# tingliu/glia

Hardware: AMD Instinct MI355X
Metric: region_merges_per_sec (higher is better)
Workload: dtype u32 labels / f32 image / f64 statistics and features

## Files before the change

### glia_amd/csrc/greedy.hip

```cpp
#include <atomic>
#include <cstring>
#include <vector>
#include <limits>
#include <rocprim/device/device_scan.hpp>
#include <rocprim/device/device_radix_sort.hpp>
#include <rocprim/device/device_segmented_radix_sort.hpp>

#include "greedy_common.hpp"

namespace glia {

__global__ void pq_build_level_kernel(PqTree t, int l) {
  const int lane = threadIdx.x & 63;
  uint32_t j = (blockIdx.x * blockDim.x + threadIdx.x) >> 6;
  if (j < t.lv[l].size) (void)pq_recompute_node(t, l, j, lane, true);
}

int pq_setup(DeviceBuffers& buf, PqTree& t, hipStream_t stream) {
  t.nlevels = 0;
  uint32_t n = t.nleaves;
  while (true) {
    n = (n + kFan - 1) / kFan;
    if (t.nlevels >= kMaxLevels) { set_error("greedy: edge table too large"); return GLIA_HMT_ERR_ARG; }
    PqLevel& L = t.lv[t.nlevels++];
// ... 881 lines not shown
          if (tid == 0) { w.cthr = (int)st.wB; w.tsal = __builtin_inf(); w.tseq = ~0ull; }
          full_barrier();
        }
      }
    }
    const int cthr2 = (wn_now + total > st.wcap) ? w.cthr : cthr;
    const double tsal2 = (wn_now + total > st.wcap) ? w.tsal : tsal;
    const unsigned long long tseq2 = (wn_now + total > st.wcap) ? w.tseq : tseq;
    const uint32_t nwork = small ? s.nitems : total;
    WPH(2);

    bool bad = false;
    uint32_t pend_e = kNone, pend_old = kNone;
    for (uint32_t base = 0; base < nwork; base += kGreedyThreads) {
      const uint32_t i = base + tid;
      if (i >= nwork) break;
      FatEntry f0, f1;
      bool h0, h1;
      uint32_t rs;
      if (small) {
        const uint32_t h = s.items[i];
        rs = s.mk[h] - 1u;
        const uint32_t m0 = s.mv0[h], m1 = s.mv1[h];
        s.mk[h] = 0u; s.mv0[h] = 0u; s.mv1[h] = 0u;
        h0 = m0 != 0; h1 = m1 != 0;
        f0 = s.stage[h0 ? m0 - 1u : m1 - 1u]; f1 = s.stage[h1 ? m1 - 1u : m0 - 1u];
      } else {
        const bool side1 = i >= len0;
        const FatEntry fe = st.fpool[side1 ? off1 + (i - len0) : off0 + i];
        if (fe.eid == e || fe.eid == kNone) continue;
        rs = fe.rs;
        if (!side1) {
          const uint32_t m = st.mark1[rs];
          h0 = true; h1 = m != 0; f0 = fe;
          f1 = h1 ? st.fpool[off1 + (m - 1u - len0)] : fe;
        } else {
          if (st.mark0[rs] != 0u) continue;
          h0 = false; h1 = true; f0 = fe; f1 = fe;
        }
      }
      const uint32_t idx = atomicAdd(&s.newcount, 1u);
      const uint32_t newE = (uint32_t)ne + idx;
      atomicOr(&w.touched[par][(rs >> 5) & 63u], 1u << (rs & 31u));
      double first = 0.0;
      int second = 0;
      if (h0) { first += f0.mean * (int)f0.n; second += (int)f0.n; }
      if (h1) { first += f1.mean * (int)f1.n; second += (int)f1.n; }
      first = sdivide(first, (double)second, 0.0);
      if (first == -1.0) bad = true;
      const uint32_t offRs = f0.off, posRs = f0.pos, lenRs = f0.len;
      if (h0 && h1) st.fpool[offRs + f1.pos].eid = kNone;
      const uint32_t cat = rs < r0 ? 0u : (h0 ? 1u : 2u);
      const unsigned long long seq = ((k + 1ull) << 32) | ((unsigned long long)cat << 30) | rs;
      const double sal = -first;
      EdgeRec* pe = &st.er[newE];
      uint4* pq4 = reinterpret_cast<uint4*>(pe);
      pq4[0] = make_uint4(rs, r2, posRs, idx);
      const unsigned long long mb = (unsigned long long)__double_as_longlong(first);
      pq4[1] = make_uint4((uint32_t)mb, (uint32_t)(mb >> 32), (uint32_t)second, kNone);
      pq4[2] = make_uint4(offRs, lenRs, r2off, 0u);
      const unsigned long long sbits = (unsigned long long)__double_as_longlong(sal);
      pq4[3] = make_uint4((uint32_t)sbits, (uint32_t)(sbits >> 32), (uint32_t)seq, (uint32_t)(seq >> 32));
      FatEntry* pa = &st.fpool[offRs + posRs];
      FatEntry a; a.eid = newE; a.rs = r2; a.n = (uint32_t)second; a.pos = idx; a.off = r2off; a.len = 0; a.mean = first;
      *pa = a;
      FatEntry b; b.eid = newE; b.rs = rs; b.n = (uint32_t)second; b.pos = posRs; b.off = offRs; b.len = lenRs; b.mean = first;
      st.fpool[r2off + idx] = b;
      if (small) { s.items[i] = offRs + posRs; s.newidx[i] = idx; }
      const uint32_t cell = win_cell(sal, smin, scale, st.wB);
      if (win_above(cthr2, tsal2, tseq2, (int)cell, sal, seq)) {
        const uint32_t sl = atomicAdd(&w.n, 1u);
        win_put(w, sl, sal, seq, newE, rs, r2, make_uint2(offRs, lenRs), make_uint2(r2off, 0u));
      } else {
        if (pend_e != kNone) st.er[pend_e].next = pend_old;
        pend_e = newE; pend_old = atomicExch(&st.whead[cell], newE);
        atomicAdd(&st.wcnt[cell], 1u);
      }
#pragma unroll
      for (int side = 0; side < 2; ++side) {
        const bool hs = side ? h1 : h0;
        if (!hs) continue;
        const uint32_t de = side ? f1.eid : f0.eid;
        const double dsal = -(side ? f1.mean : f0.mean);
        const uint32_t dc = win_cell(dsal, smin, scale, st.wB);
        unsigned long long dq = 1;
        const bool tie = (int)dc == cthr2 && dsal == tsal2;
        if (COND || tie) dq = st.er[de].seq;
        st.er[de].seq = 0;
        if (dq != 0) {
          if (win_above(cthr2, tsal2, tseq2, (int)dc, dsal, dq)) {
            const uint32_t j = atomicAdd(&w.nk, 1u); if (j < kKillMax) w.kill[j] = de; else w.kovf = 1;
          } else atomicSub(&st.wcnt[dc], 1u);
        }
      }
    }
    if (bad) s.bad = 1;
    if (small) lds_barrier(); else full_barrier();
    if (s.bad) { if (pend_e != kNone) st.er[pend_e].next = pend_old; status = ST_BAD_SALIENCY; break; }
    WPH(3);
    const uint32_t newcount = s.newcount;
    if (small) {
      for (uint32_t i = tid; i < nwork; i += kGreedyThreads) { st.fpool[s.items[i]].len = newcount; st.er[(uint32_t)ne + s.newidx[i]].hv.y = newcount; }
    } else {
      for (uint32_t j = tid; j < newcount; j += kGreedyThreads) {
        const FatEntry fb = st.fpool[r2off + j];
        st.fpool[fb.off + fb.pos].len = newcount;
        st.er[(uint32_t)ne + j].hv.y = newcount;
        st.mark0[fb.rs] = 0; st.mark1[fb.rs] = 0;
      }
    }
    if (w.kovf) full_barrier(); else lds_barrier();
    if (tid == 0) { st.adj_off[r2] = r2off; st.adj_len[r2] = newcount; s.nitems = 0; s.newcount = 0; }
    win_scan(st, w, tid, r2, newcount);
    if (pend_e != kNone) st.er[pend_e].next = pend_old;
    r2prev = r2;
    WPH(4);
#ifdef GLIA_HMT_PROFILE
    if (tid == 0) {
      const unsigned long long tn = __builtin_readcyclecounter();
      const int b = total <= 64 ? 0 : total <= 512 ? 1 : total <= kMarkMax ? 2 : total <= 8192 ? 3 : 4;
      wtb[b] += tn - wtiter; wnb[b] += 1; wdb[b] += total; wtiter = tn; winwin += w.n;
    }
#endif
    k += 1; ne += newcount; pool_used += total;
  }
#ifdef GLIA_HMT_PROFILE
  if (tid == 0) printf("[window profile] merges %llu: pop %llu  lists+table %llu  room %llu  build %llu  finish+scan %llu  loop-top %llu  reload %llu (cycles); reloads %llu (items %llu) compactions %llu dependent %llu; mean window fill %llu\n",
                       k, wph[0], wph[1], wph[2], wph[3], wph[4], wph[5], wph[6], wreloads, wloaded, wcompacts, wdeps, k ? winwin / k : 0ull);
  if (tid == 0) printf("[window profile] by width (<=64, <=512, <=1408, <=8192, more): merges %llu %llu %llu %llu %llu  cycles %llu %llu %llu %llu %llu  entries %llu %llu %llu %llu %llu\n",
                       wnb[0], wnb[1], wnb[2], wnb[3], wnb[4], wtb[0], wtb[1], wtb[2], wtb[3], wtb[4], wdb[0], wdb[1], wdb[2], wdb[3], wdb[4]);
#endif
  full_barrier();
  win_flush(st, w, tid);
  if (tid == 0) {
    st.ctrl[0] = k; st.ctrl[1] = ne; st.ctrl[2] = pool_used; st.ctrl[3] = w.err ? (unsigned long long)ST_INTERNAL : status; st.ctrl[9] = w.err; st.ctrl[10] = w.n;
    st.ctrl[5] = (unsigned long long)(long long)w.cthr; st.ctrl[6] = (unsigned long long)__double_as_longlong(w.tsal); st.ctrl[7] = w.tseq; st.ctrl[8] = w.iptr;
  }
}

constexpr uint32_t kBatchKill = 32;
constexpr int kMemP = 3;
constexpr uint32_t kMemMax = 192;
struct BatchShared {
  alignas(16) Key part1[kNW];
  alignas(16) Key part2[kNW];
  uint32_t nkill, kovf; alignas(16) uint32_t kill[kBatchKill];
  uint32_t byrank[kNW];
  uint32_t bitmap[kNW][64];
  uint32_t m_newcount[kNW], m_total[kNW], m_ok[kNW];
  double m_maxsal[kNW];
  uint32_t bad;
};

#ifdef GLIA_HMT_PROFILE
__device__ unsigned long long g_scanprof[8];
#define SCAN_T(i) do { if (tid == 0) { const unsigned long long tn_ = __builtin_readcyclecounter(); g_scanprof[i] += tn_ - st_; st_ = tn_; } } while (0)
#else
#define SCAN_T(i) do {} while (0)
#endif
__device__ __forceinline__ void batch_scan(const WinState& st, WinShared& w, BatchShared& b, int tid) {
#ifdef GLIA_HMT_PROFILE
  unsigned long long st_ = __builtin_readcyclecounter();
  if (tid == 0) g_scanprof[7] += 1;
#endif
  const uint32_t n = w.n < st.wcap ? w.n : st.wcap, nk = b.nkill < kBatchKill ? b.nkill : kBatchKill, kovf = b.kovf;
  const uint32_t own = 64u * (uint32_t)(((tid >> 6) + (tid & 63)) & 7) + (uint32_t)(tid & 63);
  unsigned long long q[kWinPer]; uint32_t e[kWinPer]; double sl[kWinPer];
#pragma unroll
  for (int j = 0; j < kWinPer; ++j) { const uint32_t i = own + (uint32_t)j * kGreedyThreads; q[j] = w.seq[i]; e[j] = w.e[i]; sl[j] = w.sal[i]; }
  const uint4 ka = *reinterpret_cast<const uint4*>(&b.kill[0]), kb = *reinterpret_cast<const uint4*>(&b.kill[4]);
  const uint32_t kl[8] = {ka.x, ka.y, ka.z, ka.w, kb.x, kb.y, kb.z, kb.w};
  Key k1, k2;
  k1.sal = -__builtin_inf(); k1.seq = 0; k1.arg = 0; k2 = k1;
  SCAN_T(0);
  uint32_t deadm[kWinPer];
#pragma unroll
  for (int j = 0; j < kWinPer; ++j) {
    uint32_t d = 0;
#pragma unroll
    for (uint32_t t = 0; t < 8; ++t) d |= (uint32_t)(t < nk) & (uint32_t)(kl[t] == e[j]);
    deadm[j] = d;
  }
  if (nk > 8u) {
    for (uint32_t t = 8; t < nk; ++t) {
      const uint32_t kt = b.kill[t];
#pragma unroll
      for (int j = 0; j < kWinPer; ++j) deadm[j] |= (uint32_t)(kt == e[j]);
    }
    if (kovf) {
      full_barrier();
#pragma unroll
      for (int j = 0; j < kWinPer; ++j) {
        const uint32_t i = own + (uint32_t)j * kGreedyThreads;
        if (i < n && q[j] != 0) deadm[j] |= (uint32_t)(st.er[e[j]].seq == 0);
      }
    }
  }
#pragma unroll
  for (int j = 0; j < kWinPer; ++j) {
    const uint32_t i = own + (uint32_t)j * kGreedyThreads;
    const bool was = (i < n) & (q[j] != 0);
    const bool live = was & (deadm[j] == 0u);
    if (was & !live) w.seq[i] = 0;
    Key c; c.sal = live ? sl[j] : -__builtin_inf(); c.seq = live ? q[j] : 0ull; c.arg = i;
    const bool b1 = better(c, k1), b2 = better(c, k2);
    k2.sal = b1 ? k1.sal : (b2 ? c.sal : k2.sal); k2.seq = b1 ? k1.seq : (b2 ? c.seq : k2.seq); k2.arg = b1 ? k1.arg : (b2 ? c.arg : k2.arg);
    k1.sal = b1 ? c.sal : k1.sal; k1.seq = b1 ? c.seq : k1.seq; k1.arg = b1 ? c.arg : k1.arg;
  }
  SCAN_T(1);
  const Key m1 = wave_max_sal_first(k1);
  SCAN_T(2);
  const bool mine = (k1.seq == m1.seq) & (k1.arg == m1.arg) & (m1.seq != 0);
  Key kk; kk.sal = mine ? k2.sal : k1.sal; kk.seq = mine ? k2.seq : k1.seq; kk.arg = mine ? k2.arg : k1.arg;
  const Key m2 = wave_max_sal_first(kk);
  SCAN_T(3);
  if ((tid & 63) == 0) { b.part1[tid >> 6] = m1; b.part2[tid >> 6] = m2; }
  full_barrier();
  SCAN_T(4);
  if (tid == 0) { b.nkill = 0; b.kovf = 0; }
}

#ifdef GLIA_HMT_PROFILE
__device__ unsigned long long g_wideprof[8];
#define WIDE_T(i) do { if (tid == 0) { const unsigned long long tn_ = __builtin_readcyclecounter(); g_wideprof[i] += tn_ - wt_; wt_ = tn_; } } while (0)
#else
#define WIDE_T(i) do {} while (0)
#endif
__device__ __forceinline__ uint32_t batch_contract_wide(const WinState& st, WinShared& w, WinWork& s, BatchShared& b, int tid, uint32_t slot, double rootsal,
                                                      unsigned long long k, unsigned long long ne, unsigned long long pool_used, uint32_t* newcount_out) {
  const double smin = st.wrange[0], scale = st.wrange[1];
  const uint32_t e = w.e[slot], r0 = w.u[slot], r1 = w.v[slot];
  const uint2 h0r = w.hu[slot], h1r = w.hv[slot];
  const uint32_t wn_now = w.n;
  const uint32_t off0 = h0r.x, len0 = h0r.y, off1 = h1r.x, len1 = h1r.y;
  const uint32_t total = len0 + len1;
  const uint32_t r2 = st.R0 + (uint32_t)k;
  const uint32_t r2off = (uint32_t)pool_used;
#ifdef GLIA_HMT_PROFILE
  unsigned long long wt_ = __builtin_readcyclecounter();
#endif
  lds_barrier();
  WIDE_T(0);
  if (tid == 0) {
    w.seq[slot] = 0;
    st.order[3 * k + 0] = r0; st.order[3 * k + 1] = r1; st.order[3 * k + 2] = r2;
    st.sal_out[k] = rootsal;
    st.er[e].seq = 0;
    st.rdead[r0] = 1; st.rdead[r1] = 1;
  }
  const bool small = total <= kMarkMax;
  for (uint32_t i = tid; i < total; i += kGreedyThreads) {
    const bool side1 = i >= len0;
    const FatEntry fe = st.fpool[side1 ? off1 + (i - len0) : off0 + i];
    if (fe.eid == e || fe.eid == kNone) continue;
    if (small) {
      s.stage[i] = fe;
      uint32_t h = (fe.rs * 2654435761u) >> 21;
      while (true) {
        const uint32_t old = atomicCAS(&s.mk[h], 0u, fe.rs + 1u);
        if (old == 0u) { s.items[atomicAdd(&s.nitems, 1u)] = h; break; }
        if (old == fe.rs + 1u) break;
        h = (h + 1u) & (kMarkSlots - 1u);
      }
      (side1 ? s.mv1 : s.mv0)[h] = i + 1u;
    } else (side1 ? st.mark1 : st.mark0)[fe.rs] = i + 1u;
  }
  if (small) lds_barrier(); else full_barrier();
  WIDE_T(1);
  if (wn_now + total > st.wcap && wn_now > st.wcap / 2u) win_compact(w, tid, st.wcap);
  WIDE_T(2);
  const int cthr = w.cthr; const double tsal = w.tsal; const unsigned long long tseq = w.tseq;
  const uint32_t nwork = small ? s.nitems : total;
  const uint32_t lenR2 = small ? nwork : 0u;
  bool bad = false;
  uint32_t pend_e = kNone, pend_old = kNone;
  auto rounds = [&](auto small_tag) {
    constexpr bool SMALL = decltype(small_tag)::value;
    for (uint32_t base = 0; base < nwork; base += kGreedyThreads) {
      const uint32_t i = base + tid;
      if (i >= nwork) break;
      FatEntry f0, f1;
      bool h0, h1;
      uint32_t rs;
      if constexpr (SMALL) {
        const uint32_t h = s.items[i];
        rs = s.mk[h] - 1u;
        const uint32_t m0 = s.mv0[h], m1 = s.mv1[h];
        s.mk[h] = 0u; s.mv0[h] = 0u; s.mv1[h] = 0u;
        h0 = m0 != 0; h1 = m1 != 0;
        f0 = s.stage[h0 ? m0 - 1u : m1 - 1u]; f1 = s.stage[h1 ? m1 - 1u : m0 - 1u];
      } else {
        const bool side1 = i >= len0;
        const FatEntry fe = st.fpool[side1 ? off1 + (i - len0) : off0 + i];
        if (fe.eid == e || fe.eid == kNone) continue;
        rs = fe.rs;
        if (!side1) {
          const uint32_t m = st.mark1[rs];
          h0 = true; h1 = m != 0; f0 = fe;
          f1 = h1 ? st.fpool[off1 + (m - 1u - len0)] : fe;
        } else {
          if (st.mark0[rs] != 0u) continue;
          h0 = false; h1 = true; f0 = fe; f1 = fe;
        }
      }
      const uint32_t idx = atomicAdd(&s.newcount, 1u);
      const uint32_t newE = (uint32_t)ne + idx;
      double first = 0.0;
      int second = 0;
      if (h0) { first += f0.mean * (int)f0.n; second += (int)f0.n; }
      if (h1) { first += f1.mean * (int)f1.n; second += (int)f1.n; }
      first = sdivide(first, (double)second, 0.0);
      if (first == -1.0) bad = true;
      const uint32_t offRs = f0.off, posRs = f0.pos, lenRs = f0.len;
      if (h0 && h1) st.fpool[offRs + f1.pos].eid = kNone;
      const uint32_t cat = rs < r0 ? 0u : (h0 ? 1u : 2u);
      const unsigned long long seq = ((k + 1ull) << 32) | ((unsigned long long)cat << 30) | rs;
      const double sal = -first;
      uint4* pq4 = reinterpret_cast<uint4*>(&st.er[newE]);
      pq4[0] = make_uint4(rs, r2, posRs, idx);
      const unsigned long long mb = (unsigned long long)__double_as_longlong(first);
      pq4[1] = make_uint4((uint32_t)mb, (uint32_t)(mb >> 32), (uint32_t)second, kNone);
      pq4[2] = make_uint4(offRs, lenRs, r2off, lenR2);
      const unsigned long long sbits = (unsigned long long)__double_as_longlong(sal);
      pq4[3] = make_uint4((uint32_t)sbits, (uint32_t)(sbits >> 32), (uint32_t)seq, (uint32_t)(seq >> 32));
      FatEntry a; a.eid = newE; a.rs = r2; a.n = (uint32_t)second; a.pos = idx; a.off = r2off; a.len = lenR2; a.mean = first;
      st.fpool[offRs + posRs] = a;
      FatEntry bb; bb.eid = newE; bb.rs = rs; bb.n = (uint32_t)second; bb.pos = posRs; bb.off = offRs; bb.len = lenRs; bb.mean = first;
      st.fpool[r2off + idx] = bb;
      const uint32_t cell = win_cell(sal, smin, scale, st.wB);
      uint32_t sl = kWinCap;
      const bool above = win_above(cthr, tsal, tseq, (int)cell, sal, seq);
      if (above) {
        sl = atomicAdd(&w.n, 1u);
        if (sl < st.wcap) win_put(w, sl, sal, seq, newE, rs, r2, make_uint2(offRs, lenRs), make_uint2(r2off, lenR2));
        else atomicMax(&w.spill_ord, f64_ord(sal));
      }
      if (sl >= st.wcap && (above || cell >= st.wch)) {
        if (pend_e != kNone) st.er[pend_e].next = pend_old;
        pend_e = newE; pend_old = atomicExch(&st.whead[cell], newE);
        atomicAdd(&st.wcnt[cell], 1u);
      }
  #pragma unroll
      for (int side = 0; side < 2; ++side) {
        const bool hs = side ? h1 : h0;
        if (!hs) continue;
        const uint32_t de = side ? f1.eid : f0.eid;
        const double dsal = -(side ? f1.mean : f0.mean);
        const uint32_t dc = win_cell(dsal, smin, scale, st.wB);
        const bool tie = (int)dc == cthr && dsal == tsal;
        if (dc >= st.wch) {
          st.er[de].seq = 0;
          if (tie || win_above(cthr, tsal, tseq, (int)dc, dsal, 0ull)) {
            const uint32_t j = atomicAdd(&b.nkill, 1u); if (j < kBatchKill) b.kill[j] = de; else b.kovf = 1;
          } else atomicSub(&st.wcnt[dc], 1u);
        }
      }
    }
  };
  if (small) rounds(std::true_type{}); else rounds(std::false_type{});
  if (bad) b.bad = 1;
  WIDE_T(3);
  if (small) lds_barrier(); else full_barrier();
  WIDE_T(4);
  const uint32_t newcount = s.newcount;
  if (!small) {
    for (uint32_t j = tid; j < newcount; j += kGreedyThreads) {
      const FatEntry fb = st.fpool[r2off + j];
      st.fpool[fb.off + fb.pos].len = newcount;
      st.er[(uint32_t)ne + j].hv.y = newcount;
      st.mark0[fb.rs] = 0; st.mark1[fb.rs] = 0;
    }
  }
  if (!small) for (uint32_t i = tid; i < (w.n < st.wcap ? w.n : st.wcap); i += kGreedyThreads) if (w.v[i] == r2) w.hv[i].y = newcount;
  if (pend_e != kNone) st.er[pend_e].next = pend_old;
  if (tid == 0) { st.adj_off[r2] = r2off; st.adj_len[r2] = newcount; }
  lds_barrier();
  WIDE_T(5);
  if (tid == 0) { s.nitems = 0; s.newcount = 0; }
  *newcount_out = newcount;
  return total;
}

__global__ __launch_bounds__(kGreedyThreads) void greedy_batch_kernel(WinState st) {
  __shared__ WinShared w;
  __shared__ WinWork s;
  __shared__ BatchShared b;
  const int tid = threadIdx.x, lane = tid & 63, wave = tid >> 6;
  unsigned long long k = st.ctrl[0], ne = st.ctrl[1], pool_used = st.ctrl[2];
  uint32_t status = ST_RUN;
  if (tid == 0) {
    w.n = 0; w.nk = 0; w.kovf = 0; w.err = 0; w.spill_ord = 0; s.nitems = 0; s.newcount = 0; s.bad = 0; b.nkill = 0; b.kovf = 0; b.bad = 0;
    w.cthr = (int)(long long)st.ctrl[5]; w.tsal = __longlong_as_double((long long)st.ctrl[6]); w.tseq = st.ctrl[7]; w.iptr = (uint32_t)st.ctrl[8];
  }
  for (uint32_t i = tid; i < kMarkSlots; i += kGreedyThreads) { s.mk[i] = 0; s.mv0[i] = 0; s.mv1[i] = 0; }
  for (uint32_t i = tid; i < kWinCap; i += kGreedyThreads) { w.seq[i] = 0; w.e[i] = 0; w.v[i] = 0; w.sal[i] = 0.0; }
  b.bitmap[wave][lane] = 0;
  if (tid < kNW) { Key z; z.sal = -__builtin_inf(); z.seq = 0; z.arg = 0; b.part1[tid] = z; b.part2[tid] = z; }
  full_barrier();
  const double smin = st.wrange[0], scale = st.wrange[1];
  uint32_t pend_e = kNone, pend_old = kNone;
  constexpr uint32_t kTab = kMarkSlots / kNW;
  uint32_t* const tk = &s.mk[wave * kTab]; uint32_t* const t0 = &s.mv0[wave * kTab]; uint32_t* const t1 = &s.mv1[wave * kTab];
  static_assert(sizeof(s.stage) >= (size_t)kNW * kTab * 20, "per-wave staging");
  uint32_t* const sg_eid = reinterpret_cast<uint32_t*>(&s.stage[0]) + wave * kTab;
  uint32_t* const sg_n = reinterpret_cast<uint32_t*>(&s.stage[0]) + (kNW + wave) * kTab;
  uint32_t* const sg_pos = reinterpret_cast<uint32_t*>(&s.stage[0]) + (2 * kNW + wave) * kTab;
  double* const sg_mean = reinterpret_cast<double*>(reinterpret_cast<uint32_t*>(&s.stage[0]) + 3 * kNW * kTab) + wave * kTab;
#ifdef GLIA_HMT_PROFILE
  unsigned long long bph[8] = {0, 0, 0, 0, 0, 0, 0, 0}, blast = __builtin_readcyclecounter(), brounds = 0, bmembers = 0, bvalid = 0, bwide = 0, bcut_sal = 0, bcut_dep = 0;
  unsigned long long bw_n[4] = {0, 0, 0, 0}, bw_cyc[4] = {0, 0, 0, 0}, bw_ent[4] = {0, 0, 0, 0}, bw_new[4] = {0, 0, 0, 0};
#define BPH(i) do { if (tid == 0) { unsigned long long tn = __builtin_readcyclecounter(); bph[i] += tn - blast; blast = tn; } } while (0)
#else
#define BPH(i) do {} while (0)
#endif

  for (unsigned long long it = 0; it < st.max_iters; ++it) {
    if (ne - st.ne_base > st.rebase_after) { status = ST_REBASE; break; }
    const int gi = lane >> 3, gj = lane & 7;
    const Key A = b.part1[gi], B = b.part1[gj], C = b.part2[gi];
    const unsigned long long beats = __ballot(better(A, B)), under = __ballot(better(C, B));
    const unsigned long long col = 0x0101010101010101ull << gj;
    const uint32_t rank = (uint32_t)__popcll(beats & col);
    const bool cand_ok = B.seq != 0 && (under & col) == 0;
    if (gi == 0 && cand_ok) b.byrank[rank] = (uint32_t)gj;
    const unsigned long long okmask = __ballot(gi == 0 && cand_ok);
    const uint32_t M = (uint32_t)__popcll(okmask);
    if (M == 0) {
      BPH(5);
      if (pend_e != kNone) { st.er[pend_e].next = pend_old; pend_e = kNone; }
      if (st.force_tree && k >= st.force_tree) { status = ST_NEED_TREE; break; }
      const int r = win_reload(st, w, tid, reinterpret_cast<double*>(&s.stage[0]), reinterpret_cast<unsigned long long*>(&s.stage[0]) + kSelMax);
      BPH(6);
      if (r == 1) { status = ST_DONE; break; }
      if (r == 2) { status = ST_NEED_TREE; break; }
      if (r == 3) { status = ST_REBASE; break; }
      batch_scan(st, w, b, tid);
      continue;
    }
    const unsigned long long minemask = __ballot(gi == 0 && cand_ok && rank == (uint32_t)wave);
    const bool member = minemask != 0;
    const int cj = member ? (int)__builtin_ctzll(minemask) : 0;
    const Key me = b.part1[cj];
    const uint32_t slot = me.arg;
    const uint32_t e = w.e[slot], r0 = w.u[slot], r1 = w.v[slot];
    const uint2 h0r = w.hu[slot], h1r = w.hv[slot];
    const uint32_t off0 = h0r.x, len0 = h0r.y, off1 = h1r.x, len1 = h1r.y;
    const uint32_t total = len0 + len1;
    if (k >= (unsigned long long)st.R0) { status = ST_INTERNAL; break; }
    const unsigned long long firstmask = __ballot(gi == 0 && cand_ok && rank == 0u);
    const Key top = b.part1[__builtin_ctzll(firstmask)];
    const uint2 th0 = w.hu[top.arg], th1 = w.hv[top.arg];
    const uint32_t top_total = th0.y + th1.y;
    BPH(0);
    if (top_total > kMemMax) {
      if (ne + top_total > st.Ecap) { status = ST_NEED_EDGES; break; }
      if (pool_used + top_total > st.pool_cap) { status = ST_NEED_POOL; break; }
      uint32_t newcount = 0;
#ifdef GLIA_HMT_PROFILE
      const unsigned long long tw0 = __builtin_readcyclecounter();
#endif
      const uint32_t tt = batch_contract_wide(st, w, s, b, tid, top.arg, top.sal, k, ne, pool_used, &newcount);
      if (b.bad) { status = ST_BAD_SALIENCY; break; }
      k += 1; ne += newcount; pool_used += tt;
#ifdef GLIA_HMT_PROFILE
      bwide += 1;
      { const int cls = tt <= 512u ? 0 : tt <= kMarkMax ? 1 : tt <= 8192u ? 2 : 3; bw_n[cls] += 1; bw_cyc[cls] += __builtin_readcyclecounter() - tw0; bw_ent[cls] += tt; bw_new[cls] += newcount; }
#endif
      batch_scan(st, w, b, tid);
      if (w.spill_ord) { if (pend_e != kNone) { st.er[pend_e].next = pend_old; pend_e = kNone; } win_evict(st, w, tid); batch_scan(st, w, b, tid); }
      BPH(4);
      continue;
    }
    const bool narrow = member && total <= kMemMax;
    b.bitmap[wave][lane] = 0;
    FatEntry fe[kMemP];
    bool act[kMemP], side1[kMemP];
    uint32_t h[kMemP];
#pragma unroll
    for (int p = 0; p < kMemP; ++p) {
      const uint32_t i = (uint32_t)lane + 64u * (uint32_t)p;
      const bool inlist = narrow && i < total;
      side1[p] = i >= len0;
      fe[p].eid = kNone; fe[p].rs = 0; fe[p].n = 0; fe[p].pos = 0; fe[p].off = 0; fe[p].len = 0; fe[p].mean = 0.0;
      if (inlist) fe[p] = st.fpool[side1[p] ? off1 + (i - len0) : off0 + i];
      act[p] = inlist;
    }
    if (pend_e != kNone) { st.er[pend_e].next = pend_old; pend_e = kNone; }
#pragma unroll
    for (int p = 0; p < kMemP; ++p) {
      act[p] = act[p] && fe[p].eid != e && fe[p].eid != kNone;
      h[p] = (fe[p].rs * 2654435761u) >> 24;
      if (act[p]) {
        while (true) {
          const uint32_t old = atomicCAS(&tk[h[p]], 0u, fe[p].rs + 1u);
          if (old == 0u || old == fe[p].rs + 1u) break;
          h[p] = (h[p] + 1u) & (kTab - 1u);
        }
        if (side1[p]) {
          t1[h[p]] = 1u;
          sg_eid[h[p]] = fe[p].eid; sg_n[h[p]] = fe[p].n; sg_pos[h[p]] = fe[p].pos; sg_mean[h[p]] = fe[p].mean;
        } else t0[h[p]] = 1u;
        atomicOr(&b.bitmap[wave][(fe[p].rs >> 5) & 63u], 1u << (fe[p].rs & 31u));
      }
    }
    if (narrow && lane == 0) { atomicOr(&b.bitmap[wave][(r0 >> 5) & 63u], 1u << (r0 & 31u)); atomicOr(&b.bitmap[wave][(r1 >> 5) & 63u], 1u << (r1 & 31u)); }
    asm volatile("s_waitcnt lgkmcnt(0)" ::: "memory");
    bool owner[kMemP], both[kMemP];
    uint32_t p_eid[kMemP], p_n[kMemP], p_pos[kMemP];
    double p_mean[kMemP];
#pragma unroll
    for (int p = 0; p < kMemP; ++p) {
      const uint32_t m0 = act[p] ? t0[h[p]] : 0u, m1 = act[p] ? t1[h[p]] : 0u;
      owner[p] = act[p] && (!side1[p] || m0 == 0u);
      both[p] = owner[p] && !side1[p] && m1 != 0u;
      p_eid[p] = sg_eid[h[p]]; p_n[p] = sg_n[h[p]]; p_pos[p] = sg_pos[h[p]]; p_mean[p] = sg_mean[h[p]];
    }
#pragma unroll
    for (int p = 0; p < kMemP; ++p) if (act[p]) { tk[h[p]] = 0u; t0[h[p]] = 0u; t1[h[p]] = 0u; }
    double first[kMemP]; int second[kMemP]; uint32_t idx[kMemP];
    bool bad = false;
    uint32_t newcount = 0;
    double mx = -__builtin_inf();
#pragma unroll
    for (int p = 0; p < kMemP; ++p) {
      const bool h0 = owner[p] && !side1[p], h1 = owner[p] && (side1[p] || both[p]);
      double f = 0.0;
      int sc = 0;
      if (h0) { f += fe[p].mean * (int)fe[p].n; sc += (int)fe[p].n; }
      if (h1) { const double m = both[p] ? p_mean[p] : fe[p].mean; const int nn = both[p] ? (int)p_n[p] : (int)fe[p].n; f += m * nn; sc += nn; }
      f = owner[p] ? sdivide(f, (double)sc, 0.0) : 0.0;
      bad = bad || (owner[p] && f == -1.0);
      first[p] = f; second[p] = sc;
      const unsigned long long ownmask = __ballot(owner[p]);
      idx[p] = newcount + (uint32_t)__popcll(ownmask & ((1ull << lane) - 1ull));
      newcount += (uint32_t)__popcll(ownmask);
      mx = (owner[p] && -f > mx) ? -f : mx;
    }
#pragma unroll
    for (int d = 32; d >= 1; d >>= 1) { const double o = __shfl_xor(mx, d); mx = o > mx ? o : mx; }
    if (lane == 0) { b.m_newcount[wave] = narrow ? newcount : 0u; b.m_total[wave] = narrow ? total : 0xFFFFFFFFu; b.m_maxsal[wave] = mx; }
    if (bad) b.bad = 1;
    const uint32_t wn_round = w.n;
    lds_barrier();
    BPH(1);
    if (b.bad) { status = ST_BAD_SALIENCY; break; }
    uint32_t V, ne_off, pool_off, my_ne, my_pool;
    {
      const uint32_t j = (uint32_t)lane & 7u;
      const Key kj = b.part1[b.byrank[j]];
      const uint32_t u = w.u[kj.arg], v = w.v[kj.arg];
      const uint32_t tj = b.m_total[j], nj = b.m_newcount[j];
      double pm = -__builtin_inf();
      uint32_t hit = 0, pre_n = 0, pre_t = 0;
#pragma unroll
      for (uint32_t i = 0; i < (uint32_t)kNW; ++i) {
        const double ms = b.m_maxsal[i];
        const uint32_t bu = b.bitmap[i][(u >> 5) & 63u], bv = b.bitmap[i][(v >> 5) & 63u];
        const uint32_t ti = b.m_total[i], ni = b.m_newcount[i];
        if (i < j) { pm = ms > pm ? ms : pm; hit |= ((bu >> (u & 31u)) | (bv >> (v & 31u))) & 1u; pre_n += ni; pre_t += ti; }
      }
      const bool okj = j < M && tj != 0xFFFFFFFFu && (j == 0u || (kj.sal > pm && hit == 0u));
      const uint32_t okbits = (uint32_t)(__ballot(lane < kNW && okj) & 0xFFull);
      V = (uint32_t)__builtin_ctz(~okbits);
#ifdef GLIA_HMT_PROFILE
      if (V < M) { const uint32_t cutsal = (uint32_t)(__ballot(lane < kNW && j == V && !(kj.sal > pm)) & 0xFFull); if (cutsal) bcut_sal += 1; else bcut_dep += 1; }
#endif
      my_ne = (uint32_t)__builtin_amdgcn_readlane((int)pre_n, wave); my_pool = (uint32_t)__builtin_amdgcn_readlane((int)pre_t, wave);
      const uint32_t last = V - 1u;
      ne_off = (uint32_t)__shfl((int)(pre_n + nj), (int)last); pool_off = (uint32_t)__shfl((int)(pre_t + tj), (int)last);
    }
    const uint32_t sum_tot = pool_off;
    if (ne + sum_tot > st.Ecap) { status = ST_NEED_EDGES; break; }
    if (pool_used + sum_tot > st.pool_cap) { status = ST_NEED_POOL; break; }
    bool popped = false;
    if (wn_round + ne_off > st.wcap && wn_round > st.wcap / 2u) {
      if ((uint32_t)wave < V && lane == 0) w.seq[slot] = 0;
      popped = true;
      lds_barrier();
      win_compact(w, tid, st.wcap);
    }
    const int cthr = w.cthr; const double tsal = w.tsal; const unsigned long long tseq = w.tseq;
    BPH(2);
    if ((uint32_t)wave < V) {
      const unsigned long long kk = k + (unsigned long long)wave;
      const uint32_t r2 = st.R0 + (uint32_t)kk;
      const uint32_t r2off = (uint32_t)pool_used + my_pool;
      if (lane == 0) {
        if (!popped) w.seq[slot] = 0;
        st.order[3 * kk + 0] = r0; st.order[3 * kk + 1] = r1; st.order[3 * kk + 2] = r2;
        st.sal_out[kk] = me.sal;
        st.er[e].seq = 0;
        st.rdead[r0] = 1; st.rdead[r1] = 1;
        st.adj_off[r2] = r2off; st.adj_len[r2] = newcount;
      }
#pragma unroll
      for (int p = 0; p < kMemP; ++p) {
        if (!owner[p]) continue;
        const bool h0 = !side1[p];
        const uint32_t rs = fe[p].rs;
        const uint32_t newE = (uint32_t)ne + my_ne + idx[p];
        const uint32_t offRs = fe[p].off, posRs = fe[p].pos, lenRs = fe[p].len;
        if (both[p]) st.fpool[offRs + p_pos[p]].eid = kNone;
        const uint32_t cat = rs < r0 ? 0u : (h0 ? 1u : 2u);
        const unsigned long long seq = ((kk + 1ull) << 32) | ((unsigned long long)cat << 30) | rs;
        const double sal = -first[p];
        uint4* pq4 = reinterpret_cast<uint4*>(&st.er[newE]);
        pq4[0] = make_uint4(rs, r2, posRs, idx[p]);
        const unsigned long long mb = (unsigned long long)__double_as_longlong(first[p]);
        pq4[1] = make_uint4((uint32_t)mb, (uint32_t)(mb >> 32), (uint32_t)second[p], kNone);
        pq4[2] = make_uint4(offRs, lenRs, r2off, newcount);
        const unsigned long long sbits = (unsigned long long)__double_as_longlong(sal);
        pq4[3] = make_uint4((uint32_t)sbits, (uint32_t)(sbits >> 32), (uint32_t)seq, (uint32_t)(seq >> 32));
        FatEntry a; a.eid = newE; a.rs = r2; a.n = (uint32_t)second[p]; a.pos = idx[p]; a.off = r2off; a.len = newcount; a.mean = first[p];
        st.fpool[offRs + posRs] = a;
        FatEntry bb; bb.eid = newE; bb.rs = rs; bb.n = (uint32_t)second[p]; bb.pos = posRs; bb.off = offRs; bb.len = lenRs; bb.mean = first[p];
        st.fpool[r2off + idx[p]] = bb;
        const uint32_t cell = win_cell(sal, smin, scale, st.wB);
        uint32_t sl = kWinCap;
        const bool above = win_above(cthr, tsal, tseq, (int)cell, sal, seq);
        if (above) {
          sl = atomicAdd(&w.n, 1u);
          if (sl < st.wcap) win_put(w, sl, sal, seq, newE, rs, r2, make_uint2(offRs, lenRs), make_uint2(r2off, newcount));
          else atomicMax(&w.spill_ord, f64_ord(sal));
        }
        if (sl >= st.wcap && (above || cell >= st.wch)) {
          if (pend_e != kNone) st.er[pend_e].next = pend_old;
          pend_e = newE; pend_old = atomicExch(&st.whead[cell], newE);
          atomicAdd(&st.wcnt[cell], 1u);
        }
#pragma unroll
        for (int side = 0; side < 2; ++side) {
          const bool hs = side ? (side1[p] || both[p]) : h0;
          if (!hs) continue;
          const uint32_t de = (side && both[p]) ? p_eid[p] : fe[p].eid;
          const double dsal = -((side && both[p]) ? p_mean[p] : fe[p].mean);
          const uint32_t dc = win_cell(dsal, smin, scale, st.wB);
          const bool tie = (int)dc == cthr && dsal == tsal;
          if (dc >= st.wch) {
            st.er[de].seq = 0;
            if (tie || win_above(cthr, tsal, tseq, (int)dc, dsal, 0ull)) {
              const uint32_t j = atomicAdd(&b.nkill, 1u); if (j < kBatchKill) b.kill[j] = de; else b.kovf = 1;
            } else atomicSub(&st.wcnt[dc], 1u);
          }
        }
      }
    }
    lds_barrier();
    BPH(3);
#ifdef GLIA_HMT_PROFILE
    brounds += 1; bmembers += M; bvalid += V;
#endif
    k += V; ne += ne_off; pool_used += pool_off;
    batch_scan(st, w, b, tid);
    if (w.spill_ord) { if (pend_e != kNone) { st.er[pend_e].next = pend_old; pend_e = kNone; } win_evict(st, w, tid); batch_scan(st, w, b, tid); }
    BPH(4);
  }
#ifdef GLIA_HMT_PROFILE
  if (tid == 0) printf("[batch profile] merges %llu: select %llu  compute %llu  validate %llu  commit %llu  scan %llu  loop-top %llu  reload %llu (cycles); rounds %llu candidates %llu committed %llu (cut by saliency %llu, by adjacency %llu) wide %llu\n",
                       k, bph[0], bph[1], bph[2], bph[3], bph[4], bph[5], bph[6], brounds, bmembers, bvalid, bcut_sal, bcut_dep, bwide);
  if (tid == 0) printf("[batch profile] scan phases (cumulative cycles, wave 0): loads %llu  compare %llu  max1 %llu  max2 %llu  barrier %llu  calls %llu\n",
                       g_scanprof[0], g_scanprof[1], g_scanprof[2], g_scanprof[3], g_scanprof[4], g_scanprof[7]);
  if (tid == 0) printf("[batch profile] wide phases (cumulative cycles): entry-barrier %llu  lists+table %llu  compact %llu  main loop (wave 0) %llu  loop barrier %llu  tail %llu\n",
                       g_wideprof[0], g_wideprof[1], g_wideprof[2], g_wideprof[3], g_wideprof[4], g_wideprof[5]);
  if (tid == 0) printf("[batch profile] wide by entries (<=512, <=1408, <=8192, more): n %llu %llu %llu %llu  cycles %llu %llu %llu %llu  entries %llu %llu %llu %llu  new edges %llu %llu %llu %llu\n",
                       bw_n[0], bw_n[1], bw_n[2], bw_n[3], bw_cyc[0], bw_cyc[1], bw_cyc[2], bw_cyc[3], bw_ent[0], bw_ent[1], bw_ent[2], bw_ent[3], bw_new[0], bw_new[1], bw_new[2], bw_new[3]);
#endif
  if (pend_e != kNone) st.er[pend_e].next = pend_old;
  full_barrier();
  win_flush(st, w, tid);
  if (tid == 0) {
    st.ctrl[0] = k; st.ctrl[1] = ne; st.ctrl[2] = pool_used; st.ctrl[3] = w.err ? (unsigned long long)ST_INTERNAL : status; st.ctrl[9] = w.err; st.ctrl[10] = w.n;
    st.ctrl[5] = (unsigned long long)(long long)w.cthr; st.ctrl[6] = (unsigned long long)__double_as_longlong(w.tsal); st.ctrl[7] = w.tseq; st.ctrl[8] = w.iptr;
  }
}

__global__ void win_range_kernel(const double* sal, uint32_t E0, unsigned long long* mm) {
  unsigned long long lo = ~0ull, hi = 0ull;
  for (uint32_t i = blockIdx.x * blockDim.x + threadIdx.x; i < E0; i += gridDim.x * blockDim.x) {
    const unsigned long long b = f64_ord(sal[i]);
    lo = b < lo ? b : lo; hi = b > hi ? b : hi;
  }
  atomicMin(&mm[0], lo); atomicMax(&mm[1], hi);
}
__global__ void win_params_kernel(const unsigned long long* mm, uint32_t B, double* range) {
  auto back = [](unsigned long long o) { o ^= (o >> 63) ? 0x8000000000000000ull : ~0ull; return __longlong_as_double((long long)o); };
  const double smin = back(mm[0]), smax = back(mm[1]);
  range[0] = smin;
  range[1] = smax > smin ? (double)B / (smax - smin) : 0.0;
}
__global__ void win_collect_kernel(const EdgeRec* er, uint32_t n_edges, const uint8_t* rdead, unsigned long long* kseq, uint32_t* vals, uint32_t* counter) {
  const uint32_t e = blockIdx.x * blockDim.x + threadIdx.x;
  if (e >= n_edges) return;
  const unsigned long long q = er[e].seq;
  if (q == 0) return;
  const uint2 uv = *reinterpret_cast<const uint2*>(&er[e].u);
  if (rdead[uv.x] | rdead[uv.y]) return;
  const uint32_t i = atomicAdd(counter, 1u);
  kseq[i] = q; vals[i] = e;
}
__global__ void win_salkey_kernel(const EdgeRec* er, const uint32_t* vals, uint32_t n, unsigned long long* ksal) {
  const uint32_t i = blockIdx.x * blockDim.x + threadIdx.x;
  if (i < n) ksal[i] = f64_ord(er[vals[i]].sal);
}
__global__ void win_baseline_fill_kernel(WinState st, uint32_t n, uint32_t* isort_w, unsigned long long* isort_seq) {
  const uint32_t i = blockIdx.x * blockDim.x + threadIdx.x;
  if (i >= n) return;
  const EdgeRec r = st.er[isort_w[i]];
  isort_seq[i] = r.seq;
  atomicAdd(&st.wcnt[win_cell(r.sal, st.wrange[0], st.wrange[1], st.wB)], 1u);
}
__global__ void win_segments_kernel(WinState st, const uint32_t* isort, uint32_t n, uint32_t* ige) {
  const uint32_t c = blockIdx.x * blockDim.x + threadIdx.x;
  if (c > st.wB) return;
  uint32_t lo = 0, hi = n;
  while (lo < hi) {
    const uint32_t mid = (lo + hi) >> 1;
    if (win_cell(st.er[isort[mid]].sal, st.wrange[0], st.wrange[1], st.wB) >= c) lo = mid + 1; else hi = mid;
  }
  ige[c] = c == 0 ? n : lo;
}
__global__ void adj_fill_fat(GreedyState g, WinState st, uint32_t E0, uint32_t* cursor) {
  const uint32_t e = blockIdx.x * blockDim.x + threadIdx.x;
  if (e >= E0) return;
  const uint32_t u = g.e_u[e], v = g.e_v[e];
  const uint32_t pu = atomicAdd(&cursor[u], 1u), pv = atomicAdd(&cursor[v], 1u);
  const uint32_t ou = g.adj_off[u], ov = g.adj_off[v], lu = g.adj_len[u], lv = g.adj_len[v];
  FatEntry a; a.eid = e; a.rs = v; a.n = (uint32_t)g.e_n[e]; a.pos = pv; a.off = ov; a.len = lv; a.mean = g.e_mean[e];
  FatEntry b = a; b.rs = u; b.pos = pu; b.off = ou; b.len = lu;
  st.fpool[ou + pu] = a; g.e_posu[e] = pu;
  st.fpool[ov + pv] = b; g.e_posv[e] = pv;
  EdgeRec r; r.u = u; r.v = v; r.posu = pu; r.posv = pv; r.mean = g.e_mean[e]; r.n = g.e_n[e]; r.next = kNone;
  r.hu = make_uint2(ou, lu); r.hv = make_uint2(ov, lv); r.sal = g.pq.leaf_sal[e]; r.seq = g.pq.leaf_seq[e];
  st.er[e] = r;
}
__global__ void fat_to_thin(const FatEntry* f, uint2* out, unsigned long long n) {
  const unsigned long long i = (unsigned long long)blockIdx.x * blockDim.x + threadIdx.x;
  if (i < n) { const FatEntry fe = f[i]; out[i] = make_uint2(fe.eid, fe.eid == kNone ? 0u : fe.rs); }
}
__global__ void edge_unpack(GreedyState g, const EdgeRec* er, const uint8_t* rdead, uint32_t n) {
  const uint32_t e = blockIdx.x * blockDim.x + threadIdx.x;
  if (e >= n) return;
  const EdgeRec r = er[e];
  g.e_u[e] = r.u; g.e_v[e] = r.v; g.e_posu[e] = r.posu; g.e_posv[e] = r.posv; g.e_mean[e] = r.mean; g.e_n[e] = r.n;
  g.pq.leaf_sal[e] = r.sal; g.pq.leaf_seq[e] = (rdead[r.u] | rdead[r.v]) ? 0ull : r.seq;
}

__global__ void edge_flags(const uint32_t* pa, const uint32_t* pb, long long P, uint32_t* flag, long long* partner) {
  long long i = (long long)blockIdx.x * blockDim.x + threadIdx.x;
  if (i >= P) return;
  uint32_t a = pa[i], b = pb[i];
  long long j = (a < b) ? find_pair(pa, pb, P, b, a) : -1;
  flag[i] = j >= 0 ? 1u : 0u;
  partner[i] = j;
}

__global__ void edge_fill(const uint32_t* pa, const uint32_t* pb, const uint32_t* prec, long long P,
                          const uint32_t* flag, const uint32_t* eidx, const long long* partner,
                          const uint32_t* rlabel, uint32_t R, GreedyState st, uint32_t* deg) {
  long long i = (long long)blockIdx.x * blockDim.x + threadIdx.x;
  if (i >= P || !flag[i]) return;
  const uint32_t e = eidx[i];
  const long long j = partner[i];
  const uint32_t u = find_label(rlabel, R, pa[i]), v = find_label(rlabel, R, pb[i]);
  const uint32_t* wi = &prec[(size_t)i * kPairWords];
  const uint32_t* wj = &prec[(size_t)j * kPairWords];
  double si, sj;
  memcpy(&si, &wi[P_SUM], 8);
  memcpy(&sj, &wj[P_SUM], 8);
  const int n = (int)(wi[P_CNT] + wj[P_CNT]);
  const double mean = sdivide(si + sj, (double)n, 0.0);
  st.e_u[e] = u; st.e_v[e] = v; st.e_mean[e] = mean; st.e_n[e] = n;
  st.pq.leaf_sal[e] = -mean; st.pq.leaf_seq[e] = (unsigned long long)e + 1ull;
  atomicAdd(&deg[u], 1u);
  atomicAdd(&deg[v], 1u);
}

__global__ void adj_fill(GreedyState st, uint32_t E0, uint32_t* cursor) {
  uint32_t e = blockIdx.x * blockDim.x + threadIdx.x;
  if (e >= E0) return;
  const uint32_t u = st.e_u[e], v = st.e_v[e];
  const uint32_t pu = atomicAdd(&cursor[u], 1u), pv = atomicAdd(&cursor[v], 1u);
  st.pool[st.adj_off[u] + pu] = make_uint2(e, v); st.e_posu[e] = pu;
  st.pool[st.adj_off[v] + pv] = make_uint2(e, u); st.e_posv[e] = pv;
}

__global__ void region_sizes(const uint32_t* rrec, uint32_t R, unsigned long long* rsz, double* rsum) {
  uint32_t r = blockIdx.x * blockDim.x + threadIdx.x;
  if (r >= R) return;
  const uint32_t* w = &rrec[(size_t)r * kRegionWords];
  rsz[r] = w[R_CNT];
  double d; memcpy(&d, &w[R_SUM], 8); rsum[r] = d;
}

__global__ void median_collect(VolumeRef vol, const uint32_t* pa, const uint32_t* pb, long long P, const uint32_t* flag,
                               const uint32_t* eidx, const unsigned long long* e_off, uint32_t* cursor, float* out) {
  const long long N = vol.nx * vol.ny * vol.nz;
  const long long p = (long long)blockIdx.x * blockDim.x + threadIdx.x;
  if (p >= N) return;
  const long long x = p % vol.nx, y = (p / vol.nx) % vol.ny, z = p / (vol.nx * vol.ny);
  const uint32_t t = vol.lab[p];
  if (t == kMaskedLabel) return;
  uint32_t nb = t;
  const long long sy = vol.nx, sz = vol.nx * vol.ny;
  const uint32_t* L = vol.lab_nb;
  do {
    uint32_t q;
    if (x > 0 && (q = L[p - 1]) != t && q != kMaskedLabel) { nb = q; break; }
    if (x + 1 < vol.nx && (q = L[p + 1]) != t && q != kMaskedLabel) { nb = q; break; }
    if (y > 0 && (q = L[p - sy]) != t && q != kMaskedLabel) { nb = q; break; }
    if (y + 1 < vol.ny && (q = L[p + sy]) != t && q != kMaskedLabel) { nb = q; break; }
    if (vol.dim == 3) {
      if (z > 0 && (q = L[p - sz]) != t && q != kMaskedLabel) { nb = q; break; }
      if (z + 1 < vol.nz && (q = L[p + sz]) != t && q != kMaskedLabel) { nb = q; break; }
    }
// ... 348 lines not shown
```

Before: 302,700.

## Specialize batch scan by window fill and use DPP top-two wave reduction

The batch scan now picks a pass instantiated for 1, 2 or 3 blocks per thread from the wave-uniform window size, so lightly filled windows skip the loads and compares for empty blocks. The two sequential key max-reductions are replaced by one DPP-based top-two reduction over ordered saliency bits. Exact ties are resolved afterwards with ballots and extra reductions on the sequence number. It also adds profiling counters for scan fill and loop-top cost. The tie handling is more complex and could differ subtly from the old ordering.

```diff
diff --git a/glia_amd/csrc/greedy.hip b/glia_amd/csrc/greedy.hip
--- a/glia_amd/csrc/greedy.hip
+++ b/glia_amd/csrc/greedy.hip
@@ -1057,68 +1057,135 @@
   uint32_t bad;
 };
 
+template <int CTRL, int ROW_MASK = 0xf>
+__device__ __forceinline__ void top2_ord_step(unsigned long long& a1, unsigned long long& a2) {
+  auto mv = [](unsigned long long v) {
+    const uint32_t lo = (uint32_t)__builtin_amdgcn_update_dpp(ROW_MASK == 0xf ? (int)(uint32_t)v : 0, (int)(uint32_t)v, CTRL, ROW_MASK, 0xf, false);
+    const uint32_t hi = (uint32_t)__builtin_amdgcn_update_dpp(ROW_MASK == 0xf ? (int)(uint32_t)(v >> 32) : 0, (int)(uint32_t)(v >> 32), CTRL, ROW_MASK, 0xf, false);
+    return ((unsigned long long)hi << 32) | lo;
+  };
+  const unsigned long long b1 = mv(a1), b2 = mv(a2);
+  const bool g = b1 > a1;
+  const unsigned long long hi = g ? b1 : a1, lo = g ? a1 : b1, m2 = b2 > a2 ? b2 : a2;
+  a1 = hi; a2 = lo > m2 ? lo : m2;
+}
+__device__ __forceinline__ void wave_top2_ord(unsigned long long& a1, unsigned long long& a2) {
+  top2_ord_step<0xB1>(a1, a2);
+  top2_ord_step<0x4E>(a1, a2);
+  top2_ord_step<0x124>(a1, a2);
+  top2_ord_step<0x128>(a1, a2);
+  top2_ord_step<0x142, 0xa>(a1, a2);
+  top2_ord_step<0x143, 0xc>(a1, a2);
+  a1 = ((unsigned long long)(uint32_t)__builtin_amdgcn_readlane((int)(uint32_t)(a1 >> 32), 63) << 32) | (uint32_t)__builtin_amdgcn_readlane((int)(uint32_t)a1, 63);
+  a2 = ((unsigned long long)(uint32_t)__builtin_amdgcn_readlane((int)(uint32_t)(a2 >> 32), 63) << 32) | (uint32_t)__builtin_amdgcn_readlane((int)(uint32_t)a2, 63);
+}
+
 #ifdef GLIA_HMT_PROFILE
 __device__ unsigned long long g_scanprof[8];
+__device__ unsigned long long g_scanfill[3][3];
 #define SCAN_T(i) do { if (tid == 0) { const unsigned long long tn_ = __builtin_readcyclecounter(); g_scanprof[i] += tn_ - st_; st_ = tn_; } } while (0)
 #else
 #define SCAN_T(i) do {} while (0)
 #endif
-__device__ __forceinline__ void batch_scan(const WinState& st, WinShared& w, BatchShared& b, int tid) {
+enum { kScanOther = 0, kScanNarrow = 1, kScanWide = 2 };
+__device__ __forceinline__ void batch_scan(const WinState& st, WinShared& w, BatchShared& b, int tid, [[maybe_unused]] int from) {
 #ifdef GLIA_HMT_PROFILE
   unsigned long long st_ = __builtin_readcyclecounter();
   if (tid == 0) g_scanprof[7] += 1;
 #endif
   const uint32_t n = w.n < st.wcap ? w.n : st.wcap, nk = b.nkill < kBatchKill ? b.nkill : kBatchKill, kovf = b.kovf;
+#ifdef GLIA_HMT_PROFILE
+  if (tid == 0) g_scanfill[from][n <= 512u ? 0 : n <= 1024u ? 1 : 2] += 1;
+#endif
   const uint32_t own = 64u * (uint32_t)(((tid >> 6) + (tid & 63)) & 7) + (uint32_t)(tid & 63);
-  unsigned long long q[kWinPer]; uint32_t e[kWinPer]; double sl[kWinPer];
-#pragma unroll
-  for (int j = 0; j < kWinPer; ++j) { const uint32_t i = own + (uint32_t)j * kGreedyThreads; q[j] = w.seq[i]; e[j] = w.e[i]; sl[j] = w.sal[i]; }
-  const uint4 ka = *reinterpret_cast<const uint4*>(&b.kill[0]), kb = *reinterpret_cast<const uint4*>(&b.kill[4]);
-  const uint32_t kl[8] = {ka.x, ka.y, ka.z, ka.w, kb.x, kb.y, kb.z, kb.w};
   Key k1, k2;
   k1.sal = -__builtin_inf(); k1.seq = 0; k1.arg = 0; k2 = k1;
-  SCAN_T(0);
-  uint32_t deadm[kWinPer];
-#pragma unroll
-  for (int j = 0; j < kWinPer; ++j) {
-    uint32_t d = 0;
-#pragma unroll
-    for (uint32_t t = 0; t < 8; ++t) d |= (uint32_t)(t < nk) & (uint32_t)(kl[t] == e[j]);
-    deadm[j] = d;
-  }
-  if (nk > 8u) {
-    for (uint32_t t = 8; t < nk; ++t) {
-      const uint32_t kt = b.kill[t];
-#pragma unroll
-      for (int j = 0; j < kWinPer; ++j) deadm[j] |= (uint32_t)(kt == e[j]);
-    }
-    if (kovf) {
-      full_barrier();
-#pragma unroll
-      for (int j = 0; j < kWinPer; ++j) {
-        const uint32_t i = own + (uint32_t)j * kGreedyThreads;
-        if (i < n && q[j] != 0) deadm[j] |= (uint32_t)(st.er[e[j]].seq == 0);
-      }
-    }
-  }
-#pragma unroll
-  for (int j = 0; j < kWinPer; ++j) {
-    const uint32_t i = own + (uint32_t)j * kGreedyThreads;
-    const bool was = (i < n) & (q[j] != 0);
-    const bool live = was & (deadm[j] == 0u);
-    if (was & !live) w.seq[i] = 0;
-    Key c; c.sal = live ? sl[j] : -__builtin_inf(); c.seq = live ? q[j] : 0ull; c.arg = i;
-    const bool b1 = better(c, k1), b2 = better(c, k2);
-    k2.sal = b1 ? k1.sal : (b2 ? c.sal : k2.sal); k2.seq = b1 ? k1.seq : (b2 ? c.seq : k2.seq); k2.arg = b1 ? k1.arg : (b2 ? c.arg : k2.arg);
-    k1.sal = b1 ? c.sal : k1.sal; k1.seq = b1 ? c.seq : k1.seq; k1.arg = b1 ? c.arg : k1.arg;
-  }
+  auto pass = [&](auto nb_tag) {
+    constexpr int NB = decltype(nb_tag)::value;
+    unsigned long long q[NB]; uint32_t e[NB]; double sl[NB];
+#pragma unroll
+    for (int j = 0; j < NB; ++j) { const uint32_t i = own + (uint32_t)j * kGreedyThreads; q[j] = w.seq[i]; e[j] = w.e[i]; sl[j] = w.sal[i]; }
+    const uint4 ka = *reinterpret_cast<const uint4*>(&b.kill[0]), kb = *reinterpret_cast<const uint4*>(&b.kill[4]);
+    const uint32_t kl[8] = {ka.x, ka.y, ka.z, ka.w, kb.x, kb.y, kb.z, kb.w};
+    SCAN_T(0);
+    uint32_t deadm[NB];
+#pragma unroll
+    for (int j = 0; j < NB; ++j) {
+      uint32_t d = 0;
+#pragma unroll
+      for (uint32_t t = 0; t < 8; ++t) d |= (uint32_t)(t < nk) & (uint32_t)(kl[t] == e[j]);
+      deadm[j] = d;
+    }
+    if (nk > 8u) {
+      for (uint32_t t = 8; t < nk; ++t) {
+        const uint32_t kt = b.kill[t];
+#pragma unroll
+        for (int j = 0; j < NB; ++j) deadm[j] |= (uint32_t)(kt == e[j]);
+      }
+      if (kovf) {
+        full_barrier();
+#pragma unroll
+        for (int j = 0; j < NB; ++j) {
+          const uint32_t i = own + (uint32_t)j * kGreedyThreads;
+          if (i < n && q[j] != 0) deadm[j] |= (uint32_t)(st.er[e[j]].seq == 0);
+        }
+      }
+    }
+#pragma unroll
+    for (int j = 0; j < NB; ++j) {
+      const uint32_t i = own + (uint32_t)j * kGreedyThreads;
+      const bool was = (i < n) & (q[j] != 0);
+      const bool live = was & (deadm[j] == 0u);
+      if (was & !live) w.seq[i] = 0;
+      Key c; c.sal = live ? sl[j] : -__builtin_inf(); c.seq = live ? q[j] : 0ull; c.arg = i;
+      const bool b1 = better(c, k1), b2 = better(c, k2);
+      k2.sal = b1 ? k1.sal : (b2 ? c.sal : k2.sal); k2.seq = b1 ? k1.seq : (b2 ? c.seq : k2.seq); k2.arg = b1 ? k1.arg : (b2 ? c.arg : k2.arg);
+      k1.sal = b1 ? c.sal : k1.sal; k1.seq = b1 ? c.seq : k1.seq; k1.arg = b1 ? c.arg : k1.arg;
+    }
+  };
+  static_assert(kWinPer == 3, "batch_scan: one pass instance per number of blocks");
+  const uint32_t nu = (uint32_t)__builtin_amdgcn_readfirstlane((int)n);
+  if (nu > 2u * kGreedyThreads) pass(std::integral_constant<int, 3>{});
+  else if (nu > kGreedyThreads) pass(std::integral_constant<int, 2>{});
+  else pass(std::integral_constant<int, 1>{});
   SCAN_T(1);
-  const Key m1 = wave_max_sal_first(k1);
-  SCAN_T(2);
-  const bool mine = (k1.seq == m1.seq) & (k1.arg == m1.arg) & (m1.seq != 0);
-  Key kk; kk.sal = mine ? k2.sal : k1.sal; kk.seq = mine ? k2.seq : k1.seq; kk.arg = mine ? k2.arg : k1.arg;
-  const Key m2 = wave_max_sal_first(kk);
-  SCAN_T(3);
+  const int lane = tid & 63;
+  const unsigned long long o1 = f64_ord(k1.sal), o2 = f64_ord(k2.sal);
+  unsigned long long M1 = o1, M2 = o2;
+  wave_top2_ord(M1, M2);
+  const unsigned long long t1 = __ballot(o1 == M1), t1l = __ballot((o1 == M1) & (k1.seq != 0ull));
+  const int l1 = (int)__builtin_ctzll(t1);
+  const bool win1 = lane == l1;
+  Key kk; kk.sal = win1 ? k2.sal : k1.sal; kk.seq = win1 ? k2.seq : k1.seq; kk.arg = win1 ? k2.arg : k1.arg;
+  const unsigned long long oc = win1 ? o2 : o1;
+  const unsigned long long t2 = __ballot(oc == M2), t2l = __ballot((oc == M2) & (kk.seq != 0ull));
+  Key m1, m2;
+  if (__popcll(t1) == 1 || t1l == 0ull) {
+    m1 = win_lane_key(k1, l1);
+    int src = (int)__builtin_ctzll(t2);
+    if (__popcll(t2) != 1 && t2l != 0ull) {
+#ifdef GLIA_HMT_PROFILE
+      if (tid == 0) g_scanprof[5] += 1;
+#endif
+      const unsigned long long ms = wave_max_u64(oc == M2 ? kk.seq : 0ull);
+      src = (int)__builtin_ctzll(__ballot((oc == M2) & (kk.seq == ms)));
+    }
+    m2 = win_lane_key(kk, src);
+    SCAN_T(2);
+  } else {
+#ifdef GLIA_HMT_PROFILE
+    if (tid == 0) g_scanprof[6] += 1;
+#endif
+    unsigned long long S1 = o1 == M1 ? k1.seq : 0ull, S2 = o2 == M1 ? k2.seq : 0ull;
+    wave_top2_ord(S1, S2);
+    const int w1 = (int)__builtin_ctzll(__ballot((o1 == M1) & (k1.seq == S1)));
+    const bool winr = lane == w1;
+    Key kc; kc.sal = winr ? k2.sal : k1.sal; kc.seq = winr ? k2.seq : k1.seq; kc.arg = winr ? k2.arg : k1.arg;
+    const unsigned long long occ = winr ? o2 : o1;
+    m1 = win_lane_key(k1, w1);
+    m2 = win_lane_key(kc, (int)__builtin_ctzll(__ballot((occ == M1) & (kc.seq == S2))));
+    SCAN_T(3);
+  }
   if ((tid & 63) == 0) { b.part1[tid >> 6] = m1; b.part2[tid >> 6] = m2; }
   full_barrier();
   SCAN_T(4);
@@ -1314,9 +1381,12 @@
 #ifdef GLIA_HMT_PROFILE
   unsigned long long bph[8] = {0, 0, 0, 0, 0, 0, 0, 0}, blast = __builtin_readcyclecounter(), brounds = 0, bmembers = 0, bvalid = 0, bwide = 0, bcut_sal = 0, bcut_dep = 0;
   unsigned long long bw_n[4] = {0, 0, 0, 0}, bw_cyc[4] = {0, 0, 0, 0}, bw_ent[4] = {0, 0, 0, 0}, bw_new[4] = {0, 0, 0, 0};
+  unsigned long long bsel[2] = {0, 0}, bsel_n[2] = {0, 0};
+#define BPH0(wide) do { if (tid == 0) { unsigned long long tn = __builtin_readcyclecounter(); bph[0] += tn - blast; bsel[wide] += tn - blast; bsel_n[wide] += 1; blast = tn; } } while (0)
 #define BPH(i) do { if (tid == 0) { unsigned long long tn = __builtin_readcyclecounter(); bph[i] += tn - blast; blast = tn; } } while (0)
 #else
 #define BPH(i) do {} while (0)
+#define BPH0(wide) do {} while (0)
 #endif
 
   for (unsigned long long it = 0; it < st.max_iters; ++it) {
@@ -1339,7 +1409,7 @@
       if (r == 1) { status = ST_DONE; break; }
       if (r == 2) { status = ST_NEED_TREE; break; }
       if (r == 3) { status = ST_REBASE; break; }
-      batch_scan(st, w, b, tid);
+      batch_scan(st, w, b, tid, kScanOther);
       continue;
     }
     const unsigned long long minemask = __ballot(gi == 0 && cand_ok && rank == (uint32_t)wave);
@@ -1356,7 +1426,7 @@
     const Key top = b.part1[__builtin_ctzll(firstmask)];
     const uint2 th0 = w.hu[top.arg], th1 = w.hv[top.arg];
     const uint32_t top_total = th0.y + th1.y;
-    BPH(0);
+    BPH0(top_total > kMemMax ? 1 : 0);
     if (top_total > kMemMax) {
       if (ne + top_total > st.Ecap) { status = ST_NEED_EDGES; break; }
       if (pool_used + top_total > st.pool_cap) { status = ST_NEED_POOL; break; }
@@ -1371,8 +1441,8 @@
       bwide += 1;
       { const int cls = tt <= 512u ? 0 : tt <= kMarkMax ? 1 : tt <= 8192u ? 2 : 3; bw_n[cls] += 1; bw_cyc[cls] += __builtin_readcyclecounter() - tw0; bw_ent[cls] += tt; bw_new[cls] += newcount; }
 #endif
-      batch_scan(st, w, b, tid);
-      if (w.spill_ord) { if (pend_e != kNone) { st.er[pend_e].next = pend_old; pend_e = kNone; } win_evict(st, w, tid); batch_scan(st, w, b, tid); }
+      batch_scan(st, w, b, tid, kScanWide);
+      if (w.spill_ord) { if (pend_e != kNone) { st.er[pend_e].next = pend_old; pend_e = kNone; } win_evict(st, w, tid); batch_scan(st, w, b, tid, kScanOther); }
       BPH(4);
       continue;
     }
@@ -1556,15 +1626,18 @@
     brounds += 1; bmembers += M; bvalid += V;
 #endif
     k += V; ne += ne_off; pool_used += pool_off;
-    batch_scan(st, w, b, tid);
-    if (w.spill_ord) { if (pend_e != kNone) { st.er[pend_e].next = pend_old; pend_e = kNone; } win_evict(st, w, tid); batch_scan(st, w, b, tid); }
+    batch_scan(st, w, b, tid, kScanNarrow);
+    if (w.spill_ord) { if (pend_e != kNone) { st.er[pend_e].next = pend_old; pend_e = kNone; } win_evict(st, w, tid); batch_scan(st, w, b, tid, kScanOther); }
     BPH(4);
   }
 #ifdef GLIA_HMT_PROFILE
   if (tid == 0) printf("[batch profile] merges %llu: select %llu  compute %llu  validate %llu  commit %llu  scan %llu  loop-top %llu  reload %llu (cycles); rounds %llu candidates %llu committed %llu (cut by saliency %llu, by adjacency %llu) wide %llu\n",
                        k, bph[0], bph[1], bph[2], bph[3], bph[4], bph[5], bph[6], brounds, bmembers, bvalid, bcut_sal, bcut_dep, bwide);
-  if (tid == 0) printf("[batch profile] scan phases (cumulative cycles, wave 0): loads %llu  compare %llu  max1 %llu  max2 %llu  barrier %llu  calls %llu\n",
-                       g_scanprof[0], g_scanprof[1], g_scanprof[2], g_scanprof[3], g_scanprof[4], g_scanprof[7]);
+  if (tid == 0) printf("[batch profile] scan phases (cumulative cycles, wave 0): loads %llu  compare %llu  top2 %llu  top2 with a tied best %llu  barrier %llu  calls %llu  tied second %llu  tied best %llu\n",
+                       g_scanprof[0], g_scanprof[1], g_scanprof[2], g_scanprof[3], g_scanprof[4], g_scanprof[7], g_scanprof[5], g_scanprof[6]);
+  if (tid == 0) printf("[batch profile] scan fill (cumulative; n <= 512, <= 1024, more): after reload/evict %llu %llu %llu  after narrow round %llu %llu %llu  after wide %llu %llu %llu\n",
+                       g_scanfill[0][0], g_scanfill[0][1], g_scanfill[0][2], g_scanfill[1][0], g_scanfill[1][1], g_scanfill[1][2], g_scanfill[2][0], g_scanfill[2][1], g_scanfill[2][2]);
+  if (tid == 0) printf("[batch profile] loop top (this launch): narrow rounds %llu cycles %llu  wide pops %llu cycles %llu\n", bsel_n[0], bsel[0], bsel_n[1], bsel[1]);
   if (tid == 0) printf("[batch profile] wide phases (cumulative cycles): entry-barrier %llu  lists+table %llu  compact %llu  main loop (wave 0) %llu  loop barrier %llu  tail %llu\n",
                        g_wideprof[0], g_wideprof[1], g_wideprof[2], g_wideprof[3], g_wideprof[4], g_wideprof[5]);
   if (tid == 0) printf("[batch profile] wide by entries (<=512, <=1408, <=8192, more): n %llu %llu %llu %llu  cycles %llu %llu %llu %llu  entries %llu %llu %llu %llu  new edges %llu %llu %llu %llu\n",
```

After: 308,200, median of 6. +1.8%, better.
